# srtee/lammps-USER-CONP2

Hardware: AMD Instinct MI355X
Metric: charge-solve updates/sec + ns/day, 4096-atom electrode / 32k electrolyte (higher is better)
Workload: dtype f64; 1 GPU; synthetic graphene/IL 4096 electrode + 32768 electrolyte, ffield; Ne=4096, Nl=32768, K=99773, kflat=645, mode=ffield, solver=inv, kspace=ewald, blist_pairs=302717, structure_factor_form=z-window (32 columns, grid 480)

## Files before the change

lammps-user-conp2_amd/csrc/conp_zn.hip:

```cpp
#include <hip/hip_runtime.h>

#include <type_traits>

#include "conp_kernels.h"

namespace conp {

typedef double d4 __attribute__((ext_vector_type(4)));
#define ZN_MFMA(a, b, c) __builtin_amdgcn_mfma_f64_16x16x4f64((a), (b), (c), 0, 0, 0)

__global__ __launch_bounds__(256) void zn_ptable_kernel(int R_pad, int C_pad, int nz, int kzt, int nzc, int n, const double *__restrict__ wfull,
                                                        const double *__restrict__ tzt , const double *__restrict__ phihat,
                                                        const double2 *__restrict__ cs, double *__restrict__ P) {
  const int g = blockIdx.x * 256 + threadIdx.x, row = blockIdx.y;
  if (g >= n) return;
  const int row_a = (row >> 6) * 128 + (row & 63);
  const double h = 6.283185307179586476925286766559 / n;
  for (int c = 0; c < nzc; ++c) {
    double s = 0.0;
    for (int m = 0; m < nz; ++m) {
      const int ct = m / kzt, ml = m - ct * kzt;
      const int cc = 320 * ct + 16 * (ml >> 3) + (ml & 7);
      const double w = wfull[(size_t)row_a * C_pad + cc];
      if (w == 0.0) continue;
      const double2 e = cs[(int)(((long long)m * g) % n)];
      s += (w / phihat[m]) * (tzt[(size_t)c * C_pad + cc] * e.x + tzt[(size_t)c * C_pad + cc + 8] * e.y);
    }
    P[(((size_t)(row >> 6) * nzc + c) * n + g) * 64 + (row & 63)] = h * s;
  }
}


constexpr int ZN_LD = 16;
#ifdef ZN_TIMELINE
__device__ unsigned long long zn_tl[8192 * 6];
__device__ unsigned long long zn_tl_chunks[16 * 64];
#define ZN_STAMP(k) do { if (threadIdx.x == 0 && blockIdx.x < 8192) zn_tl[blockIdx.x * 6 + (k)] = wall_clock64(); } while (0)
#else
#define ZN_STAMP(k) do { } while (0)
#endif
template <int NCF, bool RAW>
__global__ __launch_bounds__(256, NCF == 2 ? 4 : 3) void zn_gemm_kernel(DevPlan pl, const ZnItem *__restrict__ items, int nitems,
                                                                const double2 *__restrict__ Xt, const double2 *__restrict__ Yt,
                                                                const double *__restrict__ Bt, const double *__restrict__ P, int n, int nzc,
                                                                double *__restrict__ pieces, int piece_stride) {
  constexpr int WP = 32 * ZN_LD;
  extern __shared__ __attribute__((aligned(16))) double zn_lds[];
  ZN_STAMP(0);
#ifdef ZN_TIMELINE
  const long long zn_c0 = clock64();
#endif
  const int item_idx = (int)blockIdx.x;
  if (item_idx >= nitems) return;
  const ZnItem it = items[item_idx];
  const int t = threadIdx.x, lane = t & 63, wave = __builtin_amdgcn_readfirstlane(t >> 6);
  double *const panel0 = zn_lds + (size_t)wave * 2 * WP, *const panel1 = panel0 + WP;
  const int gj = lane & 15, g4 = lane >> 4;
  const int fr = lane & 15, fk = lane >> 4;
  const unsigned nrx16 = (unsigned)(pl.kxmax + 2) * 16, nry16 = (unsigned)(pl.kymax + 1) * 16;
  auto prow = [](int r, int a) { const int q = (r >> 1) + 8 * (r & 1); return (unsigned)(q * ZN_LD + (a ^ ((q >> 1) & 7))); };
  unsigned rdA[4];
#pragma unroll
  for (int ks = 0; ks < 4; ++ks) rdA[ks] = prow(fr, 4 * fk + ks);
  const __amdgpu_buffer_rsrc_t rx = __builtin_amdgcn_make_buffer_rsrc(const_cast<double2 *>(Xt + (size_t)it.c0 * nrx16), (short)0, -1, 0x00020000);
  const __amdgpu_buffer_rsrc_t ry = __builtin_amdgcn_make_buffer_rsrc(const_cast<double2 *>(Yt + (size_t)it.c0 * nry16), (short)0, -1, 0x00020000);
  const __amdgpu_buffer_rsrc_t rb = __builtin_amdgcn_make_buffer_rsrc(const_cast<double *>(Bt + (size_t)it.c0 * (16 * NCF * 16)), (short)0, -1, 0x00020000);
  const unsigned bby = (unsigned)((fk * 16 + fr) * 32);
  d4 acc[2][NCF];
#pragma unroll
  for (int f = 0; f < 2; ++f)
#pragma unroll
    for (int c = 0; c < NCF; ++c) acc[f][c] = (d4){0.0, 0.0, 0.0, 0.0};
  auto run = [&](auto pairedc) {
    constexpr bool PAIRED = decltype(pairedc)::value;
    constexpr int NV = PAIRED ? 2 : 4;
    unsigned xby[NV], yby[NV], sgm[NV], wa[NV], wm[NV];
#pragma unroll
    for (int u = 0; u < NV; ++u) {
      const int r = PAIRED ? 2 * (g4 + 4 * u) : g4 + 4 * u, p = it.rt * 64 + 16 * wave + r;
      xby[u] = ((unsigned)pl.p_ikx[p] * 16 + gj) * 16u; yby[u] = ((unsigned)pl.p_iky[p] * 16 + gj) * 16u;
      sgm[u] = pl.p_sgn[p] < 0 ? 0x80000000u : 0u;
      wa[u] = prow(r, gj); wm[u] = prow(r + 1, gj);
    }
    double2 X[NV], Y[NV];
    double wB[4][NCF];
    auto load_xy = [&](int u, int ch) {
      const int cr = min(ch, it.c1 - 1) - it.c0;
      X[u] = __builtin_bit_cast(double2, __builtin_amdgcn_raw_buffer_load_b128(rx, xby[u], cr * (int)(nrx16 * 16), 0));
      Y[u] = __builtin_bit_cast(double2, __builtin_amdgcn_raw_buffer_load_b128(ry, yby[u], cr * (int)(nry16 * 16), 0));
    };
    auto load_w = [&](int half, int ch) {
      const int cr = min(ch, it.c1 - 1) - it.c0;
#pragma unroll
      for (int c = 0; c < NCF; ++c) {
        const double2 v = __builtin_bit_cast(double2, __builtin_amdgcn_raw_buffer_load_b128(rb, bby + 2048 * c + 16 * half, cr * (16 * NCF * 16 * 8), 0));
        wB[2 * half][c] = v.x; wB[2 * half + 1][c] = v.y;
      }
    };
#pragma unroll
    for (int u = 0; u < NV; ++u) load_xy(u, it.c0);
#pragma unroll
    for (int u = 0; u < NV; ++u) {
      if constexpr (PAIRED) {
        const double t2 = X[u].y * Y[u].y, t4 = X[u].y * Y[u].x;
        panel0[wa[u]] = X[u].x * Y[u].x - t2; panel0[wm[u]] = X[u].x * Y[u].x + t2;
        panel0[wa[u] + 16 * ZN_LD] = X[u].x * Y[u].y + t4; panel0[wm[u] + 16 * ZN_LD] = t4 - X[u].x * Y[u].y;
      } else {
        const double sy = __hiloint2double(__double2hiint(Y[u].y) ^ (int)sgm[u], __double2loint(Y[u].y));
        panel0[wa[u]] = X[u].x * Y[u].x - X[u].y * sy;
        panel0[wa[u] + 16 * ZN_LD] = X[u].x * sy + X[u].y * Y[u].x;
      }
    }
#pragma unroll
    for (int u = 0; u < NV; ++u) {
      load_xy(u, it.c0 + 1);
      if (u == NV / 2 - 1) load_w(0, it.c0);
    }
    load_w(1, it.c0);
    ZN_STAMP(1);
    double fa[2][2];
    auto frag = [&](const double *pn, int ks, int set) { fa[set][0] = pn[rdA[ks]]; fa[set][1] = pn[rdA[ks] + 16 * ZN_LD]; };
    frag(panel0, 0, 0);
    auto chunk = [&](int ch, auto bufc) {
      constexpr int BUF = decltype(bufc)::value;
      const double *pn = BUF ? panel1 : panel0;
      double *pw = BUF ? panel0 : panel1;
      double sy = 0.0, va = 0.0, vb = 0.0, vc = 0.0, vd = 0.0, t2 = 0.0, t4 = 0.0;
#pragma unroll
      for (int ks = 0; ks < 4; ++ks) {
        const int cur = ks & 1, nx = cur ^ 1;
        frag(ks < 3 ? pn : pw, ks < 3 ? ks + 1 : 0, nx);
        __builtin_amdgcn_sched_barrier(0);
#pragma unroll
        for (int m = 0; m < 2 * NCF; ++m) {
          const int f = m & 1, c = m >> 1;
          acc[f][c] = ZN_MFMA(wB[ks][c], fa[cur][f], acc[f][c]);
          const int g = 4 * ks + m;
          if (ks < 3 && m < 4) {
            if constexpr (PAIRED) {
              const int u = g / 6, part = g - 6 * u;
              if (part == 0) { t2 = X[u].y * Y[u].y; va = X[u].x * Y[u].x - t2; }
              else if (part == 1) vb = X[u].x * Y[u].x + t2;
              else if (part == 2) { t4 = X[u].y * Y[u].x; vc = X[u].x * Y[u].y + t4; }
              else if (part == 3) vd = t4 - X[u].x * Y[u].y;
              else if (part == 4) { pw[wa[u]] = va; pw[wm[u]] = vb; pw[wa[u] + 16 * ZN_LD] = vc; pw[wm[u] + 16 * ZN_LD] = vd; }
              else load_xy(u, ch + 2);
            } else {
              const int u = g / 3, part = g - 3 * u;
              if (part == 0) {
                sy = __hiloint2double(__double2hiint(Y[u].y) ^ (int)sgm[u], __double2loint(Y[u].y));
                va = X[u].x * Y[u].x - X[u].y * sy;
              } else if (part == 1) vb = X[u].x * sy + X[u].y * Y[u].x;
              else { pw[wa[u]] = va; pw[wa[u] + 16 * ZN_LD] = vb; load_xy(u, ch + 2); }
            }
          }
          __builtin_amdgcn_sched_barrier(0);
        }
        if (ks & 1) { load_w(ks >> 1, ch + 1); __builtin_amdgcn_sched_barrier(0); }
      }
#ifdef ZN_TIMELINE
      if (t == 0 && (blockIdx.x & 255) == 0 && (blockIdx.x >> 8) < 16 && ch - it.c0 < 64) zn_tl_chunks[(blockIdx.x >> 8) * 64 + ch - it.c0] = wall_clock64();
#endif
    };
    const int nmax = it.c1 - it.c0;
#ifndef ZN_SKIP_MAIN
    for (int i = 0; i < nmax; i += 2) {
      chunk(it.c0 + i, std::integral_constant<int, 0>());
      if (i + 1 < nmax) chunk(it.c0 + i + 1, std::integral_constant<int, 1>());
    }
#endif
  };
  if (it.paired) run(std::true_type()); else run(std::false_type());
  ZN_STAMP(2);
  if constexpr (RAW) {
    double *raw = pieces + (size_t)it.slot * (16 * NCF * 128) + 16 * wave + fr;
#pragma unroll
    for (int f = 0; f < 2; ++f)
#pragma unroll
      for (int cf = 0; cf < NCF; ++cf)
#pragma unroll
        for (int r = 0; r < 4; ++r) raw[(16 * cf + 4 * r + fk) * 128 + 64 * f] = acc[f][cf][r];
    return;
  }
  double *out = pieces + (size_t)it.slot * piece_stride + 16 * wave + fr;
  unsigned gofs[NCF][4];
#pragma unroll
  for (int cf = 0; cf < NCF; ++cf)
#pragma unroll
    for (int r = 0; r < 4; ++r) { int g = (it.g0 + 16 * cf + 4 * r + fk) % n; gofs[cf][r] = (unsigned)(g < 0 ? g + n : g) * 64u; }
  const double *Pw = P + (size_t)it.rt * nzc * n * 64 + 16 * wave + fr;
  constexpr int CB = 3;
#ifdef ZN_SKIP_EPI
  for (int cb = 0; cb < 1; cb += CB) {
#else
  for (int cb = 0; cb < nzc; cb += CB) {
#endif
    double pv[CB][NCF][4];
#pragma unroll
    for (int k = 0; k < CB; ++k) {
      const double *pc = Pw + (size_t)min(cb + k, nzc - 1) * n * 64;
#pragma unroll
      for (int cf = 0; cf < NCF; ++cf)
#pragma unroll
        for (int r = 0; r < 4; ++r) pv[k][cf][r] = pc[gofs[cf][r]];
    }
#pragma unroll
    for (int k = 0; k < CB; ++k) {
      double s0 = 0.0, s1 = 0.0;
#pragma unroll
      for (int cf = 0; cf < NCF; ++cf)
#pragma unroll
        for (int r = 0; r < 4; ++r) { s0 += acc[0][cf][r] * pv[k][cf][r]; s1 += acc[1][cf][r] * pv[k][cf][r]; }
      s0 += __shfl_xor(s0, 16, 64); s1 += __shfl_xor(s1, 16, 64);
      s0 += __shfl_xor(s0, 32, 64); s1 += __shfl_xor(s1, 32, 64);
      if (fk == 0 && cb + k < nzc) { out[(cb + k) * 128] = s0; out[(cb + k) * 128 + 64] = s1; }
    }
  }
#ifdef ZN_TIMELINE
  __syncthreads();
  ZN_STAMP(3);
  if (threadIdx.x == 0 && blockIdx.x < 8192) {
    unsigned hw, xcc;
    asm volatile("s_getreg_b32 %0, hwreg(HW_REG_HW_ID)" : "=s"(hw));
    asm volatile("s_getreg_b32 %0, hwreg(HW_REG_XCC_ID)" : "=s"(xcc));
    zn_tl[blockIdx.x * 6 + 4] = ((unsigned long long)xcc << 32) | hw;
    zn_tl[blockIdx.x * 6 + 5] = (unsigned long long)(it.c1 - it.c0) | ((unsigned long long)(clock64() - zn_c0) << 16);
  }
#endif
}

void launch_zn_ptable(hipStream_t s, const DevPlan &pl, int kzt, int nzc, int n, const double *tzt, const double *phihat, const double2 *cs,
                      double *P) {
  hipLaunchKernelGGL(zn_ptable_kernel, dim3((n + 255) / 256, pl.R_pad / 2), dim3(256), 0, s, pl.R_pad, pl.C_pad, pl.nz, kzt, nzc, n, pl.wfull, tzt,
                     phihat, cs, P);
}
template <int NCF, bool RAW>
static void zn_gemm_launch(hipStream_t s, const DevPlan &pl, const ZnItem *items, int nitems, const double2 *Xt, const double2 *Yt,
                           const double *Bt, const double *P, int n, int nzc, double *pieces, int piece_stride) {
  constexpr int lds = 4 * 2 * 32 * ZN_LD * 8;
  const int nblocks = (nitems + 7) / 8 * 8;
  hipLaunchKernelGGL((zn_gemm_kernel<NCF, RAW>), dim3(nblocks), dim3(256), lds, s, pl, items, nitems, Xt, Yt, Bt, P, n, nzc, pieces,
                     piece_stride);
}
void launch_zn_gemm(hipStream_t s, const DevPlan &pl, int ncf, const ZnItem *items, int nitems, const double2 *Xt, const double2 *Yt,
                    const double *Bt, const double *P, int n, int nzc, double *pieces, int piece_stride) {
  if (nitems <= 0) return;
  if (P == nullptr) {
    if (ncf == 2) zn_gemm_launch<2, true>(s, pl, items, nitems, Xt, Yt, Bt, P, n, nzc, pieces, piece_stride);
    else zn_gemm_launch<3, true>(s, pl, items, nitems, Xt, Yt, Bt, P, n, nzc, pieces, piece_stride);
  } else if (ncf == 2) zn_gemm_launch<2, false>(s, pl, items, nitems, Xt, Yt, Bt, P, n, nzc, pieces, piece_stride);
  else zn_gemm_launch<3, false>(s, pl, items, nitems, Xt, Yt, Bt, P, n, nzc, pieces, piece_stride);
}

__global__ __launch_bounds__(128) void zn_wsum_kernel(int n, int nrg, int ncol, const int *__restrict__ cov_ptr, const int2 *__restrict__ cov_ent,
                                                      const double *__restrict__ raw, double *__restrict__ grid) {
  const int g = blockIdx.x, k = blockIdx.y, row = threadIdx.x;
  double s = 0.0;
  const int e0 = cov_ptr[g], e1 = cov_ptr[g + 1];
  for (int e = e0; e < e1; e += 4) {
    double v[4];
#pragma unroll
    for (int u = 0; u < 4; ++u) {
      const int2 en = cov_ent[min(e + u, e1 - 1)];
      v[u] = raw[((size_t)(k * nrg + en.x) * ncol + en.y) * 128 + row];
      if (e + u >= e1) v[u] = 0.0;
    }
    s += (v[0] + v[1]) + (v[2] + v[3]);
  }
  grid[((size_t)k * n + g) * 128 + row] = s;
}
__global__ __launch_bounds__(256) void zn_dtable_kernel(int C_pad, int nz, int kzt, int n, const double *__restrict__ phihat,
                                                        const double2 *__restrict__ cs, double *__restrict__ Dt) {
  const int col = blockIdx.x * 256 + threadIdx.x, g = blockIdx.y;
  if (col >= C_pad) return;
  const int ct = col / 320, cl = col - 320 * ct;
  const int ml = 8 * (cl >> 4) + (cl & 7), m = ct * kzt + ml;
  double v = 0.0;
  if (ml < kzt && m < nz) {
    const double2 e = cs[(int)(((long long)m * g) % n)];
    v = (6.283185307179586476925286766559 / n / phihat[m]) * ((cl & 8) ? e.y : e.x);
  }
  Dt[(size_t)g * C_pad + col] = v;
}
__global__ __launch_bounds__(256) void zn_dft_kernel(int n, int C_pad, int nz, int kzt, const int *__restrict__ own_rt, const double *__restrict__ grid,
                                                     const double *__restrict__ Dt, const double *__restrict__ wfull, double *__restrict__ G,
                                                     double *__restrict__ Gwf) {
  __shared__ double part[3][64][16];
  const int lane = threadIdx.x & 63, fr = lane & 15, fk = lane >> 4, kq = threadIdx.x >> 6;
  const int k = blockIdx.x >> 2, fp = blockIdx.x & 3, rt = own_rt[k], cb0 = 2 * blockIdx.y;
  {
    const int ct = 16 * cb0 / 320, ml0 = 8 * ((16 * cb0 - 320 * ct) >> 4);
    if (ml0 >= kzt || ct * kzt + ml0 >= nz) return;
  }
  const int nkq = n / 16, kbeg = kq * nkq, nks = kbeg + nkq;
  const double *a = grid + ((size_t)k * n + fk) * 128 + 32 * fp + fr;
  const double *b = Dt + (size_t)fk * C_pad + 16 * cb0 + fr;
  d4 acc[2][2];
#pragma unroll
  for (int i = 0; i < 2; ++i)
#pragma unroll
    for (int j = 0; j < 2; ++j) acc[i][j] = (d4){0.0, 0.0, 0.0, 0.0};
  constexpr int KB = 8;
  double a0[KB][2], b0[KB][2], a1[KB][2], b1[KB][2];
  auto fetch = [&](double(*av)[2], double(*bv)[2], int k0) {
#pragma unroll
    for (int i = 0; i < KB; ++i) {
      const int ks = min(k0 + i, nks - 1);
      av[i][0] = a[(size_t)ks * 512]; av[i][1] = a[(size_t)ks * 512 + 16];
      bv[i][0] = b[(size_t)ks * 4 * C_pad]; bv[i][1] = b[(size_t)ks * 4 * C_pad + 16];
    }
  };
  auto mult = [&](const double(*av)[2], const double(*bv)[2], int k0) {
#pragma unroll
    for (int i = 0; i < KB; ++i) {
      const bool on = k0 + i < nks;
      const double x0 = on ? av[i][0] : 0.0, x1 = on ? av[i][1] : 0.0;
      acc[0][0] = ZN_MFMA(x0, bv[i][0], acc[0][0]); acc[0][1] = ZN_MFMA(x0, bv[i][1], acc[0][1]);
      acc[1][0] = ZN_MFMA(x1, bv[i][0], acc[1][0]); acc[1][1] = ZN_MFMA(x1, bv[i][1], acc[1][1]);
    }
  };
  fetch(a0, b0, kbeg);
  for (int k0 = kbeg; k0 < nks; k0 += 2 * KB) {
    fetch(a1, b1, k0 + KB);
    mult(a0, b0, k0);
    fetch(a0, b0, k0 + 2 * KB);
    mult(a1, b1, k0 + KB);
  }
  if (kq > 0) {
#pragma unroll
    for (int i = 0; i < 2; ++i)
#pragma unroll
      for (int j = 0; j < 2; ++j)
#pragma unroll
        for (int r = 0; r < 4; ++r) part[kq - 1][lane][(2 * i + j) * 4 + r] = acc[i][j][r];
  }
  __syncthreads();
  if (kq > 0) return;
#pragma unroll
  for (int i = 0; i < 2; ++i)
#pragma unroll
    for (int j = 0; j < 2; ++j) {
      const int f16 = 2 * fp + i, gcol = 16 * (cb0 + j) + fr;
      const size_t rf = (size_t)rt * 8 + f16;
#pragma unroll
      for (int r = 0; r < 4; ++r) {
        const double v = ((acc[i][j][r] + part[0][lane][(2 * i + j) * 4 + r]) + part[1][lane][(2 * i + j) * 4 + r]) + part[2][lane][(2 * i + j) * 4 + r];
        const int row16 = 4 * r + fk;
        const size_t grow = (size_t)rt * 128 + 16 * f16 + row16;
        G[grow * C_pad + gcol] = v;
        Gwf[(rf * (C_pad / 4) + (gcol >> 2)) * 64 + (gcol & 3) * 16 + row16] = wfull[grow * C_pad + gcol] * v;
      }
    }
}
void launch_zn_dtable(hipStream_t s, const DevPlan &pl, int kzt, int n, const double *phihat, const double2 *cs, double *Dt) {
  hipLaunchKernelGGL(zn_dtable_kernel, dim3((pl.C_pad + 255) / 256, n), dim3(256), 0, s, pl.C_pad, pl.nz, kzt, n, phihat, cs, Dt);
}
void launch_zn_windows_to_g(hipStream_t s, const DevPlan &pl, int kzt, int n, int n_own, const int *own_rt, int nrg, int ncol, const int *cov_ptr,
                            const int2 *cov_ent, const double *raw, double *grid, const double *Dt, double *G, double *Gwf) {
  hipLaunchKernelGGL(zn_wsum_kernel, dim3(n, n_own), dim3(128), 0, s, n, nrg, ncol, cov_ptr, cov_ent, raw, grid);
  hipLaunchKernelGGL(zn_dft_kernel, dim3(4 * n_own, pl.C_pad / 32), dim3(256), 0, s, n, pl.C_pad, pl.nz, kzt, own_rt, grid, Dt, pl.wfull, G, Gwf);
}

}

#ifdef ZN_TIMELINE
extern "C" int conp_debug_zn_timeline(unsigned long long *out, int nblocks) {
  return (int)hipMemcpyFromSymbol(out, HIP_SYMBOL(conp::zn_tl), sizeof(unsigned long long) * 6 * (size_t)nblocks);
}
extern "C" int conp_debug_zn_timeline_chunks(unsigned long long *out) {
  return (int)hipMemcpyFromSymbol(out, HIP_SYMBOL(conp::zn_tl_chunks), sizeof(unsigned long long) * 16 * 64);
}
#endif
```

Before: 11480 updates/s.

## Peel last GEMM chunk to prefetch P-table loads and pipeline epilogue batches

Peels the final chunk of the z-window MFMA loop into a specialized LAST variant that skips the next-panel staging and weight prefetch. It issues the epilogue's P-table buffer loads during those last MFMAs instead. The epilogue now uses buffer loads with precomputed wrapped offsets and software-pipelines the next batch of P values while the current batch is reduced. The goal is to hide the latency of the first and later P-table loads behind compute. In exchange it adds register pressure from the pv/pofs arrays and a host-side guard that n is at least one window long.

```diff
diff --git a/lammps-user-conp2_amd/csrc/conp_zn.hip b/lammps-user-conp2_amd/csrc/conp_zn.hip
--- a/lammps-user-conp2_amd/csrc/conp_zn.hip
+++ b/lammps-user-conp2_amd/csrc/conp_zn.hip
@@ -1,5 +1,6 @@
 #include <hip/hip_runtime.h>
 
+#include <stdexcept>
 #include <type_traits>
 
 #include "conp_kernels.h"
@@ -71,6 +72,21 @@
   for (int f = 0; f < 2; ++f)
 #pragma unroll
     for (int c = 0; c < NCF; ++c) acc[f][c] = (d4){0.0, 0.0, 0.0, 0.0};
+  constexpr int CB = 3;
+  const double *Pw = nullptr;
+  __amdgpu_buffer_rsrc_t rp = rx;
+  unsigned pbase = 0, pnb = 0, pso[CB] = {};
+  unsigned pofs[NCF][4];
+  double pv[CB][NCF][4];
+  if constexpr (!RAW) {
+    int gb = it.g0 % n;
+    gb = __builtin_amdgcn_readfirstlane(gb < 0 ? gb + n : gb);
+    Pw = P + (size_t)it.rt * nzc * n * 64 + 16 * wave;
+    rp = __builtin_amdgcn_make_buffer_rsrc(const_cast<double *>(Pw), (short)0, -1, 0x00020000);
+    pbase = ((unsigned)(gb + fk) * 64u + (unsigned)fr) * 8u; pnb = (unsigned)n * 512u;
+#pragma unroll
+    for (int k = 0; k < CB; ++k) pso[k] = __builtin_amdgcn_readfirstlane((unsigned)max(min(k, nzc - 1), 0) * pnb);
+  }
   auto run = [&](auto pairedc) {
     constexpr bool PAIRED = decltype(pairedc)::value;
     constexpr int NV = PAIRED ? 2 : 4;
@@ -90,7 +106,7 @@
       Y[u] = __builtin_bit_cast(double2, __builtin_amdgcn_raw_buffer_load_b128(ry, yby[u], cr * (int)(nry16 * 16), 0));
     };
     auto load_w = [&](int half, int ch) {
-      const int cr = min(ch, it.c1 - 1) - it.c0;
+      const int cr = ch - it.c0;
 #pragma unroll
       for (int c = 0; c < NCF; ++c) {
         const double2 v = __builtin_bit_cast(double2, __builtin_amdgcn_raw_buffer_load_b128(rb, bby + 2048 * c + 16 * half, cr * (16 * NCF * 16 * 8), 0));
@@ -121,22 +137,35 @@
     double fa[2][2];
     auto frag = [&](const double *pn, int ks, int set) { fa[set][0] = pn[rdA[ks]]; fa[set][1] = pn[rdA[ks] + 16 * ZN_LD]; };
     frag(panel0, 0, 0);
-    auto chunk = [&](int ch, auto bufc) {
+    const int nfull = it.c1 - it.c0 - 1;
+    auto chunk = [&](int ch, auto bufc, auto lastc) {
       constexpr int BUF = decltype(bufc)::value;
-      const double *pn = BUF ? panel1 : panel0;
+      constexpr bool LAST = decltype(lastc)::value;
+      const double *pn = LAST ? ((nfull & 1) ? panel1 : panel0) : BUF ? panel1 : panel0;
       double *pw = BUF ? panel0 : panel1;
       double sy = 0.0, va = 0.0, vb = 0.0, vc = 0.0, vd = 0.0, t2 = 0.0, t4 = 0.0;
 #pragma unroll
       for (int ks = 0; ks < 4; ++ks) {
         const int cur = ks & 1, nx = cur ^ 1;
-        frag(ks < 3 ? pn : pw, ks < 3 ? ks + 1 : 0, nx);
+        if (!(LAST && ks == 3)) frag(ks < 3 ? pn : pw, ks < 3 ? ks + 1 : 0, nx);
         __builtin_amdgcn_sched_barrier(0);
 #pragma unroll
         for (int m = 0; m < 2 * NCF; ++m) {
           const int f = m & 1, c = m >> 1;
           acc[f][c] = ZN_MFMA(wB[ks][c], fa[cur][f], acc[f][c]);
           const int g = 4 * ks + m;
-          if (ks < 3 && m < 4) {
+          if constexpr (LAST) {
+            if constexpr (!RAW) {
+              if (ks < 3 && m < 4 && g < 4 * NCF) {
+                const int cf = g >> 2, r = g & 3;
+                const unsigned o = pbase + (unsigned)(16 * cf + 4 * r) * 512u;
+                pofs[cf][r] = min(o, o - pnb);
+#pragma unroll
+                for (int k = 0; k < CB; ++k)
+                  pv[k][cf][r] = __builtin_bit_cast(double, __builtin_amdgcn_raw_buffer_load_b64(rp, pofs[cf][r], pso[k], 0));
+              }
+            }
+          } else if (ks < 3 && m < 4) {
             if constexpr (PAIRED) {
               const int u = g / 6, part = g - 6 * u;
               if (part == 0) { t2 = X[u].y * Y[u].y; va = X[u].x * Y[u].x - t2; }
@@ -156,18 +185,20 @@
           }
           __builtin_amdgcn_sched_barrier(0);
         }
-        if (ks & 1) { load_w(ks >> 1, ch + 1); __builtin_amdgcn_sched_barrier(0); }
+        if (!LAST && (ks & 1)) { load_w(ks >> 1, ch + 1); __builtin_amdgcn_sched_barrier(0); }
       }
 #ifdef ZN_TIMELINE
       if (t == 0 && (blockIdx.x & 255) == 0 && (blockIdx.x >> 8) < 16 && ch - it.c0 < 64) zn_tl_chunks[(blockIdx.x >> 8) * 64 + ch - it.c0] = wall_clock64();
 #endif
     };
-    const int nmax = it.c1 - it.c0;
 #ifndef ZN_SKIP_MAIN
-    for (int i = 0; i < nmax; i += 2) {
-      chunk(it.c0 + i, std::integral_constant<int, 0>());
-      if (i + 1 < nmax) chunk(it.c0 + i + 1, std::integral_constant<int, 1>());
-    }
+    constexpr std::integral_constant<int, 0> b0{};
+    constexpr std::integral_constant<int, 1> b1{};
+    for (int i = 0; i < nfull; i += 2) {
+      chunk(it.c0 + i, b0, std::false_type());
+      if (i + 1 < nfull) chunk(it.c0 + i + 1, b1, std::false_type());
+    }
+    if (nfull >= 0) chunk(it.c1 - 1, b0, std::true_type());
 #endif
   };
   if (it.paired) run(std::true_type()); else run(std::false_type());
@@ -183,27 +214,30 @@
     return;
   }
   double *out = pieces + (size_t)it.slot * piece_stride + 16 * wave + fr;
-  unsigned gofs[NCF][4];
-#pragma unroll
-  for (int cf = 0; cf < NCF; ++cf)
-#pragma unroll
-    for (int r = 0; r < 4; ++r) { int g = (it.g0 + 16 * cf + 4 * r + fk) % n; gofs[cf][r] = (unsigned)(g < 0 ? g + n : g) * 64u; }
-  const double *Pw = P + (size_t)it.rt * nzc * n * 64 + 16 * wave + fr;
-  constexpr int CB = 3;
+#ifdef ZN_SKIP_MAIN
+  {
+#else
+  if (it.c1 <= it.c0) {
+#endif
+#pragma unroll
+    for (int cf = 0; cf < NCF; ++cf)
+#pragma unroll
+      for (int r = 0; r < 4; ++r) {
+        const unsigned o = pbase + (unsigned)(16 * cf + 4 * r) * 512u;
+        pofs[cf][r] = min(o, o - pnb);
+#pragma unroll
+        for (int k = 0; k < CB; ++k) pv[k][cf][r] = __builtin_bit_cast(double, __builtin_amdgcn_raw_buffer_load_b64(rp, pofs[cf][r], pso[k], 0));
+      }
+  }
 #ifdef ZN_SKIP_EPI
-  for (int cb = 0; cb < 1; cb += CB) {
+  const int ncls = min(nzc, CB);
 #else
-  for (int cb = 0; cb < nzc; cb += CB) {
-#endif
-    double pv[CB][NCF][4];
-#pragma unroll
-    for (int k = 0; k < CB; ++k) {
-      const double *pc = Pw + (size_t)min(cb + k, nzc - 1) * n * 64;
-#pragma unroll
-      for (int cf = 0; cf < NCF; ++cf)
-#pragma unroll
-        for (int r = 0; r < 4; ++r) pv[k][cf][r] = pc[gofs[cf][r]];
-    }
+  const int ncls = nzc;
+#endif
+  auto batch = [&](int cb, auto morec) {
+    constexpr bool MORE = decltype(morec)::value;
+    __amdgpu_buffer_rsrc_t rn = rp;
+    if constexpr (MORE) rn = __builtin_amdgcn_make_buffer_rsrc(const_cast<double *>(Pw + (size_t)(cb + CB) * n * 64), (short)0, -1, 0x00020000);
 #pragma unroll
     for (int k = 0; k < CB; ++k) {
       double s0 = 0.0, s1 = 0.0;
@@ -211,11 +245,21 @@
       for (int cf = 0; cf < NCF; ++cf)
 #pragma unroll
         for (int r = 0; r < 4; ++r) { s0 += acc[0][cf][r] * pv[k][cf][r]; s1 += acc[1][cf][r] * pv[k][cf][r]; }
+      if constexpr (MORE) {
+        const unsigned so = __builtin_amdgcn_readfirstlane((unsigned)min(k, ncls - 1 - cb - CB) * pnb);
+#pragma unroll
+        for (int cf = 0; cf < NCF; ++cf)
+#pragma unroll
+          for (int r = 0; r < 4; ++r) pv[k][cf][r] = __builtin_bit_cast(double, __builtin_amdgcn_raw_buffer_load_b64(rn, pofs[cf][r], so, 0));
+      }
       s0 += __shfl_xor(s0, 16, 64); s1 += __shfl_xor(s1, 16, 64);
       s0 += __shfl_xor(s0, 32, 64); s1 += __shfl_xor(s1, 32, 64);
-      if (fk == 0 && cb + k < nzc) { out[(cb + k) * 128] = s0; out[(cb + k) * 128 + 64] = s1; }
-    }
-  }
+      if (fk == 0 && cb + k < ncls) { out[(cb + k) * 128] = s0; out[(cb + k) * 128 + 64] = s1; }
+    }
+  };
+  int cb = 0;
+  for (; cb + CB < ncls; cb += CB) batch(cb, std::true_type());
+  if (cb < ncls) batch(cb, std::false_type());
 #ifdef ZN_TIMELINE
   __syncthreads();
   ZN_STAMP(3);
@@ -245,6 +289,7 @@
 void launch_zn_gemm(hipStream_t s, const DevPlan &pl, int ncf, const ZnItem *items, int nitems, const double2 *Xt, const double2 *Yt,
                     const double *Bt, const double *P, int n, int nzc, double *pieces, int piece_stride) {
   if (nitems <= 0) return;
+  if (P != nullptr && n < 16 * ncf) throw std::invalid_argument("zn_gemm: the z grid is shorter than a window");
   if (P == nullptr) {
     if (ncf == 2) zn_gemm_launch<2, true>(s, pl, items, nitems, Xt, Yt, Bt, P, n, nzc, pieces, piece_stride);
     else zn_gemm_launch<3, true>(s, pl, items, nitems, Xt, Yt, Bt, P, n, nzc, pieces, piece_stride);
```

Result: faster. 11720 updates/s (median of 6 runs) (+2.1%).
